# Mange/raingun

Hardware: AMD Instinct MI355X
Metric: Mrays/sec (primary+shadow+secondary) at 3840×2160, depth 5; 1/2/4/8 MI355X (higher is better)
Workload: dtype f64

## Files before the change

include/raingun_debug.h:

```cpp
#ifndef RAINGUN_DEBUG_H
#define RAINGUN_DEBUG_H

#include "raingun.h"

#ifdef __cplusplus
extern "C" {
#endif

rg_status rg_debug_set_path(rg_scene *scene, int32_t path);

typedef struct rg_bvh_info {
    int32_t built;
    int32_t enabled;
    int32_t nodes;
    int32_t leaves;
    int32_t depth;
    float margin;
    float origin_bound;
    int32_t lane_stack;
    int64_t lbuf_bytes;
} rg_bvh_info;
rg_status rg_debug_set_bvh(rg_scene *scene, int32_t enable);
rg_status rg_debug_bvh_info(const rg_scene *scene, rg_bvh_info *info);

// ... 15 lines not shown

rg_status rg_debug_set_host_tile_shape(rg_scene *scene, int32_t tile_wlog);

rg_status rg_debug_set_aa_band_rows(rg_scene *scene, int32_t rows);

rg_status rg_debug_set_aa_adaptive_timing(rg_scene *scene, int32_t enable);
rg_status rg_debug_aa_adaptive_info(const rg_scene *scene, float ms[5], uint32_t *flagged, uint32_t *listed_tiles,
                                    uint32_t *bands_launched);

rg_status rg_debug_set_multi(rg_scene *scene, int32_t mode, int32_t stand_in, int32_t bands, int32_t only_rank);

int rg_debug_gather_noop(const void *send, void *recv, size_t count, int datatype, int root, void *comm,
                         void *stream);

rg_status rg_debug_counters(const rg_scene *scene, uint64_t out[16]);

rg_status rg_debug_counter_words(const rg_scene *scene, int32_t first, int32_t n, uint64_t *out);

rg_status rg_debug_last_plain(const rg_scene *scene, int32_t *plain);

typedef struct rg_shadow_volume_info {
    int32_t built;
    int32_t enabled;
    int32_t g;
    int32_t pad;
    int64_t bytes;
    double build_ms;
    double set_share;
} rg_shadow_volume_info;
rg_status rg_debug_set_shadow_volume(rg_scene *scene, int32_t on);
rg_status rg_debug_shadow_volume_info(const rg_scene *scene, rg_shadow_volume_info *info);
rg_status rg_debug_last_shadow_volume(const rg_scene *scene, int32_t *used);

rg_status rg_debug_set_exact_div(rg_scene *scene, int32_t enable);
rg_status rg_debug_camera_check(const rg_scene *scene, uint32_t width, uint32_t height, double fov,
                                uint64_t *mismatches, int32_t *admitted);

rg_status rg_debug_unscaled_check(const rg_scene *scene, int32_t op, const double *a, const double *b, uint32_t n,
                                  uint64_t *mismatches);

#ifdef __cplusplus
}
#endif

#endif
```

raingun_amd/_abi.py:

```python
from __future__ import annotations

import ctypes as C
import os
from pathlib import Path

PKG_DIR = Path(__file__).resolve().parent
REPO_DIR = PKG_DIR.parent
LIB_PATH = PKG_DIR / "libraingun_hip.so"

RG_OK = 0
RG_ERR_INVALID_ARGUMENT = -1
RG_ERR_PORTRAIT = -2
RG_ERR_AABB_NORMAL = -3
RG_ERR_NAN_DISTANCE = -4
RG_ERR_TRANSMISSION = -5
RG_ERR_TEXTURE = -6
RG_ERR_DEVICE = -10
RG_ERR_OUT_OF_MEMORY = -11
RG_ERR_CANCELLED = -12
RG_ERR_COLLECTIVE = -13
RG_ERR_PENDING = -14

BODY_SPHERE, BODY_PLANE, BODY_DISK, BODY_AABB = 0, 1, 2, 3
COLORATION_COLOR, COLORATION_TEXTURE = 0, 1
# ... 112 lines not shown
    "rg_scene_set_max_depth",
    "rg_render_image",
    "rg_render_tiles_async",
    "rg_render_tiles_pipelined",
    "rg_render_tiles",
    "rg_tiling_rows",
    "rg_render_stream",
    "rg_trace",
    "rg_host_register",
    "rg_host_unregister",
    "rg_scene_release_stream",
    "rg_stream_status",
    "rg_render_multi",
    "rg_render_image_aa",
    "rg_render_aa_async",
    "rg_resolve_box",
    "rg_render_image_aa_adaptive",
    "rg_render_aa_adaptive",
    "rg_edge_mask",
    "rg_camera_look_at",
    "rg_scene_set_camera",
    "rg_render_aov",
    "rg_render_aov_async",
    "rg_scene_set_lens",
    "rg_lens_tables",
)
DEBUG_SYMBOLS = ("rg_debug_set_path", "rg_debug_set_bvh", "rg_debug_bvh_info", "rg_debug_counters",
                 "rg_debug_set_lightbuf", "rg_debug_lightbuf_count",
                 "rg_debug_set_tile_order", "rg_debug_set_lane_depth", "rg_debug_set_image_bands", "rg_debug_set_host_split",
                 "rg_debug_fail_split_a", "rg_debug_set_host_ring", "rg_debug_set_host_tile_shape", "rg_debug_set_multi", "rg_debug_gather_noop",
                 "rg_debug_counter_words", "rg_debug_set_aa_band_rows",
                 "rg_debug_set_aa_adaptive_timing", "rg_debug_aa_adaptive_info", "rg_debug_last_plain",
                 "rg_debug_set_shadow_volume", "rg_debug_shadow_volume_info", "rg_debug_last_shadow_volume",
                 "rg_debug_set_exact_div", "rg_debug_camera_check", "rg_debug_unscaled_check")
FRAMES_SYMBOLS = ("rg_frames_create", "rg_frames_destroy", "rg_frames_step", "rg_frames_flush", "rg_frames_image",
                  "rg_frames_read_image", "rg_frames_status", "rg_frames_set_batch", "rg_frames_set_root_tiles", "rg_comm_id_bytes",
                  "rg_comm_unique_id", "rg_comm_init_rank", "rg_comm_info", "rg_comm_destroy", "rg_comm_gather_fn")
PATH_AUTO, PATH_LIGHT, PATH_HEAVY = -1, 0, 1


class RaingunError(RuntimeError):

    def __init__(self, status: int, what: str = ""):
        self.status = status
        msg = status_string(status) if _LIB is not None else str(status)
        super().__init__(f"{what}: {msg} (status {status})" if what else f"{msg} (status {status})")


_LIB: C.CDLL | None = None


def _declare(lib: C.CDLL) -> None:
    P = C.POINTER
    lib.rg_abi_version.restype = C.c_int32
    lib.rg_status_string.restype = C.c_char_p
    lib.rg_status_string.argtypes = [C.c_int32]
    lib.rg_device_count.restype = C.c_int32
    lib.rg_scene_create.restype = C.c_int32
    lib.rg_scene_create.argtypes = [P(rg_scene_desc), C.c_int32, P(C.c_void_p)]
    lib.rg_scene_destroy.restype = None
    lib.rg_scene_destroy.argtypes = [C.c_void_p]
    lib.rg_scene_set_max_depth.restype = C.c_int32
    lib.rg_scene_set_max_depth.argtypes = [C.c_void_p, C.c_uint32]
    lib.rg_camera_look_at.restype = C.c_int32
    lib.rg_camera_look_at.argtypes = [P(C.c_double), P(C.c_double), P(C.c_double), P(rg_camera)]
    lib.rg_scene_set_camera.restype = C.c_int32
# ... 36 lines not shown
    lib.rg_debug_set_lane_depth.argtypes = [C.c_void_p, C.c_int32]
    lib.rg_debug_set_image_bands.restype = C.c_int32
    lib.rg_debug_set_image_bands.argtypes = [C.c_void_p, C.c_int32]
    if hasattr(lib, "rg_debug_set_host_split"):
        lib.rg_debug_set_host_split.restype = C.c_int32
        lib.rg_debug_set_host_split.argtypes = [C.c_void_p, C.c_int32]
    if hasattr(lib, "rg_debug_set_host_ring"):
        lib.rg_debug_set_host_ring.restype = C.c_int32
        lib.rg_debug_set_host_ring.argtypes = [C.c_void_p] + [C.c_int32] * 5
    if hasattr(lib, "rg_debug_fail_split_a"):
        lib.rg_debug_fail_split_a.restype = C.c_int32
        lib.rg_debug_fail_split_a.argtypes = [C.c_void_p, C.c_int32]
    if hasattr(lib, "rg_debug_set_multi"):
        lib.rg_debug_set_multi.restype = C.c_int32
        lib.rg_debug_set_multi.argtypes = [C.c_void_p, C.c_int32, C.c_int32, C.c_int32, C.c_int32]
    if hasattr(lib, "rg_debug_set_host_tile_shape"):
        lib.rg_debug_set_host_tile_shape.restype = C.c_int32
        lib.rg_debug_set_host_tile_shape.argtypes = [C.c_void_p, C.c_int32]
    lib.rg_debug_counters.restype = C.c_int32
    lib.rg_debug_counters.argtypes = [C.c_void_p, P(C.c_uint64)]
    if hasattr(lib, "rg_debug_counter_words"):
        lib.rg_debug_counter_words.restype = C.c_int32
        lib.rg_debug_counter_words.argtypes = [C.c_void_p, C.c_int32, C.c_int32, P(C.c_uint64)]
    if hasattr(lib, "rg_debug_last_plain"):
        lib.rg_debug_last_plain.restype = C.c_int32
        lib.rg_debug_last_plain.argtypes = [C.c_void_p, P(C.c_int32)]
    if hasattr(lib, "rg_debug_set_shadow_volume"):
        lib.rg_debug_set_shadow_volume.restype = C.c_int32
        lib.rg_debug_set_shadow_volume.argtypes = [C.c_void_p, C.c_int32]
        lib.rg_debug_shadow_volume_info.restype = C.c_int32
        lib.rg_debug_shadow_volume_info.argtypes = [C.c_void_p, P(rg_shadow_volume_info)]
        lib.rg_debug_last_shadow_volume.restype = C.c_int32
        lib.rg_debug_last_shadow_volume.argtypes = [C.c_void_p, P(C.c_int32)]
    if hasattr(lib, "rg_debug_set_exact_div"):
        lib.rg_debug_set_exact_div.restype = C.c_int32
        lib.rg_debug_set_exact_div.argtypes = [C.c_void_p, C.c_int32]
        lib.rg_debug_camera_check.restype = C.c_int32
        lib.rg_debug_camera_check.argtypes = [C.c_void_p, C.c_uint32, C.c_uint32, C.c_double, P(C.c_uint64), P(C.c_int32)]
    if hasattr(lib, "rg_debug_unscaled_check"):
        lib.rg_debug_unscaled_check.restype = C.c_int32
        lib.rg_debug_unscaled_check.argtypes = [C.c_void_p, C.c_int32, C.c_void_p, C.c_void_p, C.c_uint32, P(C.c_uint64)]
    lib.rg_frames_create.restype = C.c_int32
    lib.rg_frames_create.argtypes = [C.c_void_p, C.c_uint32, C.c_uint32, C.c_uint32, C.c_int32, C.c_int32,
                                     C.c_int32, C.c_void_p, C.c_void_p, P(C.c_void_p)]
    lib.rg_frames_destroy.restype = None
    lib.rg_frames_destroy.argtypes = [C.c_void_p]
    lib.rg_frames_step.restype = C.c_int32
    lib.rg_frames_step.argtypes = [C.c_void_p]
    lib.rg_frames_flush.restype = C.c_int32
    lib.rg_frames_flush.argtypes = [C.c_void_p]
    lib.rg_frames_image.restype = C.c_void_p
    lib.rg_frames_image.argtypes = [C.c_void_p]
    lib.rg_frames_read_image.restype = C.c_int32
    lib.rg_frames_read_image.argtypes = [C.c_void_p, C.c_void_p]
    lib.rg_trace.restype = C.c_int32
    lib.rg_trace.argtypes = [C.c_void_p, C.c_void_p, C.c_uint32, C.c_void_p, C.c_void_p]
    lib.rg_host_register.restype = C.c_int32
    lib.rg_host_register.argtypes = [C.c_void_p, C.c_size_t]
    lib.rg_host_unregister.restype = C.c_int32
    lib.rg_host_unregister.argtypes = [C.c_void_p]
    lib.rg_scene_release_stream.restype = C.c_int32
    lib.rg_scene_release_stream.argtypes = [C.c_void_p, C.c_void_p]
    lib.rg_stream_status.restype = C.c_int32
    lib.rg_stream_status.argtypes = [C.c_void_p, C.c_void_p, P(C.c_int32)]
    lib.rg_render_multi.restype = C.c_int32
    lib.rg_render_multi.argtypes = [C.c_void_p, C.c_uint32, C.c_uint32, C.c_int32, C.c_uint32, C.c_void_p,
# ... 100 lines not shown
```

raingun_amd/csrc/rg_capi.hip:

```cpp
#include <hip/hip_runtime.h>

#include <algorithm>
#include <cstring>

#include "../../include/raingun.h"
#include "../../include/raingun_debug.h"
#include "rg_device.h"
#include "rg_exact.h"
#include "rg_internal.h"
#include "rg_launchers.h"

#pragma clang fp contract(off)

#ifndef RG_LANE_MIN_DEPTH
#define RG_LANE_MIN_DEPTH 1
#endif

void rg_image_res_release(rg_image_res &r) {
    rg_bands_release(r);
    if (r.h_frame) (void)hipHostFree(r.h_frame);
    if (r.h_flags) (void)hipHostFree(r.h_flags);
    if (r.h_cancel) (void)hipHostFree(r.h_cancel);
    r = rg_image_res{};
}
// ... 425 lines not shown
    if (!s || !out) return RG_ERR_INVALID_ARGUMENT;
    if (!ok(hipSetDevice(s->device))) return RG_ERR_DEVICE;
    if (!ok(hipStreamSynchronize(s->last->stream)) ||
        !ok(hipMemcpy(out, s->last->last_counters, 16 * sizeof(uint64_t), hipMemcpyDeviceToHost)))
        return RG_ERR_DEVICE;
    return RG_OK;
}

rg_status rg_debug_last_plain(const rg_scene *s, int32_t *plain) {
    if (!s || !plain || !s->last) return RG_ERR_INVALID_ARGUMENT;
    *plain = s->last->last_plain;
    return RG_OK;
}

rg_status rg_debug_set_shadow_volume(rg_scene *s, int32_t on) {
    if (!s || (on != 0 && on != 1)) return RG_ERR_INVALID_ARGUMENT;
    s->shvol_enabled = on != 0;
    return RG_OK;
}

rg_status rg_debug_shadow_volume_info(const rg_scene *s, rg_shadow_volume_info *info) {
    if (!s || !info) return RG_ERR_INVALID_ARGUMENT;
    *info = s->shvol_info;
    info->enabled = s->shvol_info.built && s->shvol_enabled;
    return RG_OK;
}

rg_status rg_debug_last_shadow_volume(const rg_scene *s, int32_t *used) {
    if (!s || !used || !s->last) return RG_ERR_INVALID_ARGUMENT;
    *used = s->last->last_shvol;
    return RG_OK;
}

rg_status rg_debug_set_exact_div(rg_scene *s, int32_t enable) {
    if (!s || (enable != 0 && enable != 1)) return RG_ERR_INVALID_ARGUMENT;
    s->exact_div = enable != 0;
    return RG_OK;
}

rg_status rg_debug_camera_check(const rg_scene *s, uint32_t width, uint32_t height, double fov, uint64_t *mismatches,
                                int32_t *admitted) {
    if (!s || !mismatches || width == 0 || height == 0 || (unsigned long long)width * height >= (1ull << 32))
        return RG_ERR_INVALID_ARGUMENT;
    if (!ok(hipSetDevice(s->device))) return RG_ERR_DEVICE;
    RgKernelArgs a = rg_make_args(s);
    a.width = width;
    a.height = height;
    a.width_d = (double)width;
    a.height_d = (double)height;
    a.aspect = a.width_d / a.height_d;
    a.fov_adjustment = rg_fov_adjustment(fov);
    a.inv_w = 1.0 / a.width_d;
    a.inv_h = 1.0 / a.height_d;
    if (admitted)
        *admitted = rg_recip_div_ok(width) && rg_recip_div_ok(height) && rg_camera_unscaled_ok(a.fov_adjustment, a.aspect);
    unsigned long long *d_bad = nullptr, bad = 0;
    if (!ok(hipMalloc(&d_bad, sizeof bad))) return RG_ERR_OUT_OF_MEMORY;
    rg_status st = RG_OK;
    if (!ok(hipMemset(d_bad, 0, sizeof bad)) || !ok(rg_launch_camera_check(&a, d_bad, nullptr)) ||
        !ok(hipMemcpy(&bad, d_bad, sizeof bad, hipMemcpyDeviceToHost)))
        st = RG_ERR_DEVICE;
    (void)hipFree(d_bad);
    *mismatches = bad;
    return st;
}

// ... 66 lines not shown
```

raingun_amd/csrc/rg_device.h:

```cpp
#pragma once
#include <stdint.h>

#if !defined(__HIP__) && !defined(__HIPCC__)
#define __device__
#define __host__
#define __forceinline__ inline
#endif

#ifdef __HIP_DEVICE_COMPILE__
#define RG_CONST __attribute__((address_space(4)))
#else
#define RG_CONST
#endif
template <class T>
__device__ __forceinline__ const RG_CONST T *rg_cptr(const T *p) { return (const RG_CONST T *)p; }

struct alignas(16) RgSph { double cx, cy, cz, r2; };
struct alignas(16) RgSphF { float cx, cy, cz, r2hi; };
struct alignas(16) RgSphF2 { float cchi, thrp, cc32; int32_t id; };
struct alignas(16) RgPln { double ox, oy, oz, nx, ny, nz, on, pad; };
struct alignas(16) RgDsk { double ox, oy, oz, nx, ny, nz, r, on; };
struct alignas(16) RgBox { double lo[3], hi[3]; };

struct alignas(16) RgBvhNode {
// ... 95 lines not shown
    int32_t nan_scene;
    unsigned long long *err_sticky;
    uint32_t *tile_flags;
    uint32_t frame_seq;
    const uint32_t *cancel;
    uint32_t tile_wlog;
    uint32_t defer_px;
    const double *prim_sx, *prim_sy;
    uint32_t pipelined;
    double width_d, height_d;
    unsigned long long *snap_out;
    uint32_t max_grid_threads;
    uint32_t image_rows;
    uint32_t out_tile_mul, out_tile_add;
    const void *lds_blob;
    const RgLightBufDev *lbuf;
    const uint32_t *lb_start;
    const uint32_t *lb_ent;
    int32_t n_lbuf;
    int32_t lb_cam;
    uint32_t lds_lbuf;
    uint32_t ring_flush, ring_group;
    const uint8_t *px_mask;
    uint32_t tile_limit, px_k, px_w;
    uint32_t plain_veto;
    double inv_w, inv_h;
    uint32_t tiles_x_m, tiles_x_sh, tile_rows_shift, tile_rows_m, tile_rows_sh, rows_identity;
    uint32_t lds_texm, lds_axes, lds_plain_bytes;
    uint32_t camera;
    double cam_eye[3], cam_right[3], cam_up[3], cam_forward[3];
    const uint32_t *shvol;
    uint32_t shvol_g;
    float shvol_inv, shvol_off;
    uint32_t shvol_pad[3];
    uint32_t lens, lens_k;
    double lens_focus, lens_r[3], lens_u[3];
    const double *lens_tab;
    uint32_t lens_pad[2];
};

__host__ __device__ inline uint32_t rg_tile_w(const RgKernelArgs &a) { return 1u << a.tile_wlog; }
__host__ __device__ inline uint32_t rg_tile_h(const RgKernelArgs &a) { return 64u >> a.tile_wlog; }
__host__ __device__ inline uint32_t rg_tiles_x(const RgKernelArgs &a) { return (a.width + rg_tile_w(a) - 1u) >> a.tile_wlog; }
__host__ __device__ inline uint32_t rg_tiles_y(const RgKernelArgs &a) { return (a.out_rows + rg_tile_h(a) - 1u) / rg_tile_h(a); }
__host__ __device__ inline unsigned long long rg_tile_count(const RgKernelArgs &a) {
    return (unsigned long long)rg_tiles_x(a) * rg_tiles_y(a);
}

#define RG_FRAME_BYTES 88

#ifndef RG_RING_FLUSH_SMALL
#define RG_RING_FLUSH_SMALL 4
#endif
#ifndef RG_RING_GROUP_SMALL
#define RG_RING_GROUP_SMALL 1
#endif
#ifndef RG_RING_FLUSH_BIG
#define RG_RING_FLUSH_BIG 8
#endif
#ifndef RG_RING_GROUP_BIG
#define RG_RING_GROUP_BIG 8
#endif
#ifndef RG_RING_BIG_TILES
#define RG_RING_BIG_TILES 50000u
#endif
#ifndef RG_MULTI_LIGHT_ONE
#define RG_MULTI_LIGHT_ONE 1
#endif
#ifndef RG_LB
#define RG_LB 3
#endif
#ifndef RG_LB_SMALL
#define RG_LB_SMALL 2
#endif
#ifndef RG_LB_ONE
#define RG_LB_ONE 1
#endif
#ifndef RG_PLAIN_SHVOL
#define RG_PLAIN_SHVOL 1
#endif
#ifndef RG_PLAIN_SHVOL_SPHERES
#define RG_PLAIN_SHVOL_SPHERES 1
#endif
#ifndef RG_PLAIN_SHVOL_PLANES
#define RG_PLAIN_SHVOL_PLANES 1
#endif
#ifndef RG_HEAVY_WPS
#define RG_HEAVY_WPS 3
#endif
#define RG_BVH_MAX_WAVES 16
#ifndef RG_HEAVY_SCENE_BODIES
#define RG_HEAVY_SCENE_BODIES 32
#endif

#define RG_PATH_AUTO -1
#define RG_PATH_LIGHT 0
#define RG_PATH_HEAVY 1

__host__ __device__ __forceinline__ bool rg_heavy_path(const RgKernelArgs &a) {
    bool heavy = a.n_sph + a.n_pln + a.n_dsk + a.n_box >= RG_HEAVY_SCENE_BODIES;
    if (a.path != RG_PATH_AUTO) heavy = a.path == RG_PATH_HEAVY;
    if (a.n_lights > RG_LB) heavy = true;
    return heavy;
}

#define RG_COUNTER_WORDS (16 + 16 * 16 + 16)
#define RG_DONE_WORD (16 + 16 * 16)
```

raingun_amd/csrc/rg_internal.h:

```cpp
#pragma once
#include <hip/hip_runtime.h>

#include <cstddef>
#include <cstring>
#include <initializer_list>
#include <memory>
#include <vector>

#include "../../include/raingun.h"
#include "../../include/raingun_debug.h"
#include "rg_bands.h"
#include "rg_copy_pool.h"
#include "rg_device.h"
#include "rg_lightbuf_ray.h"
#include "rg_tile_deal.h"

inline bool ok(hipError_t e) { return e == hipSuccess; }

struct rg_launch_ctx {
    hipStream_t stream = nullptr;
    unsigned long long *counters = nullptr;
    int cur = 0;
    unsigned long long *last_counters = nullptr;
    int last_plain = 0;
// ... 99 lines not shown
    int device = 0;
    double fov = 90.0;
    float def[3] = {0, 0, 0};
    uint32_t max_depth = 10;
    int32_t n_sph = 0, n_pln = 0, n_dsk = 0, n_box = 0, n_bodies = 0, n_lights = 0, n_textures = 0;
    bool nan_scene = false;
    std::vector<void *> allocations;
    RgSph *sph = nullptr;
    double *sph_cc = nullptr;
    RgSphF *sphf = nullptr;
    RgSphF2 *sphf2 = nullptr;
    int32_t path = RG_PATH_AUTO;
    int32_t *sph_id = nullptr, *pln_id = nullptr, *dsk_id = nullptr, *box_id = nullptr;
    RgPln *pln = nullptr;
    RgDsk *dsk = nullptr;
    RgBox *box = nullptr;
    RgBodyDev *bodies = nullptr;
    RgMatDev *mats = nullptr;
    RgLightDev *lights = nullptr;
    RgTexDev *texs = nullptr;
    RgBvhNode *nodes = nullptr;
    int32_t n_nodes = 0;
    int32_t lane_stack = 0;
    int32_t lane_min_depth = 1;
    bool bvh_enabled = true;
    RgLightBufDev *lbuf = nullptr;
    uint32_t *lb_start = nullptr, *lb_ent = nullptr;
    int32_t n_lbuf = 0;
    int32_t lb_cam = -1;
    int32_t n_lbdesc = 0;
    bool lbuf_enabled = true;
    uint32_t *shvol = nullptr;
    bool shvol_enabled = true;
    rg_shadow_volume_info shvol_info{};
    float shvol_inv = 0.0f, shvol_off = 0.0f;
    bool exact_div = true;
    bool has_camera = false;
    rg_camera camera{};
    rg_lens lens{0.0, 1.0};
    float bvh_obound = 0.0f;
    double bvh_rbound = 0.0, bvh_margin = 0.0, bvh_extent = 0.0;
    rg_bvh_info bvh_info{};
    int tile_order = -1;
    int image_bands = 0;
    int host_split_pct = 0;
    mutable int split_fail_a = 0;
    int ring_flush_small = RG_RING_FLUSH_SMALL, ring_group_small = RG_RING_GROUP_SMALL;
    int ring_flush_big = RG_RING_FLUSH_BIG, ring_group_big = RG_RING_GROUP_BIG;
    bool multi_light_one = RG_MULTI_LIGHT_ONE != 0;
    int host_tile_wlog = RG_HOST_TILE_WLOG;
    bool host_tile_forced = false;
    int multi_mode = 0;
    bool multi_stand_in = false;
    int multi_bands = 0;
    int multi_only_rank = -1;
    std::shared_ptr<const rg_host_tables> host;
    std::vector<RgTexDev> tex_desc;
    void *lds_blob = nullptr;
    uint32_t lds_blob_layout[14] = {};
    mutable std::vector<rg_launch_ctx *> ctxs;
    mutable rg_launch_ctx *last = nullptr;
    mutable rg_image_res img;
    int aa_band_rows = 0;
    mutable rg_aa_res aa;
    mutable rg_multi_res *multi = nullptr;
    mutable std::vector<rg_frames *> frames;
// ... 81 lines not shown
```

raingun_amd/csrc/rg_k_math.h:

```cpp
#pragma once
#include <hip/hip_runtime.h>
#include <cstdint>

#include "rg_device.h"
#include "rg_exact.h"

#pragma clang fp contract(off)

namespace rgk {

constexpr double SHADOW_BIAS = 1e-13;
constexpr float PI_F = 3.14159265358979323846f;

enum : int { MODE_CLOSEST = 0, MODE_SHADOW = 1, MODE_DONE = 2, MODE_WAIT = 3, MODE_SHADOW_H = 4 };
enum : int { FR_REFL = 0, FR_REFR_T = 1, FR_REFR_R = 2, FR_REFR_TASK = 4, FR_REFR_WAIT = 5 };

struct V3 { double x, y, z; };
struct C3 { float r, g, b; };

__device__ __forceinline__ V3 v3(double x, double y, double z) { return V3{x, y, z}; }
__device__ __forceinline__ V3 add(V3 a, V3 b) { return v3(a.x + b.x, a.y + b.y, a.z + b.z); }
__device__ __forceinline__ V3 sub(V3 a, V3 b) { return v3(a.x - b.x, a.y - b.y, a.z - b.z); }
__device__ __forceinline__ V3 scl(V3 a, double s) { return v3(a.x * s, a.y * s, a.z * s); }
__device__ __forceinline__ V3 neg(V3 a) { return v3(-a.x, -a.y, -a.z); }
// ... 76 lines not shown
__device__ __forceinline__ C3 cadd(C3 a, C3 b) { return c3(a.r + b.r, a.g + b.g, a.b + b.b); }
__device__ __forceinline__ C3 cmul(C3 a, C3 b) { return c3(a.r * b.r, a.g * b.g, a.b * b.b); }
__device__ __forceinline__ C3 cscl(C3 a, float s) { return c3(a.r * s, a.g * s, a.b * s); }
__device__ __forceinline__ C3 cclamp(C3 a) {
    return c3(fmaxf(fminf(a.r, 1.0f), 0.0f), fmaxf(fminf(a.g, 1.0f), 0.0f), fmaxf(fminf(a.b, 1.0f), 0.0f));
}

__device__ __forceinline__ uint32_t f32_to_u8(float v) {
    if (!(v > 0.0f)) return 0u;
    if (v >= 255.0f) return 255u;
    return (uint32_t)v;
}
__device__ __forceinline__ int32_t f32_to_i32(float v) {
    if (v != v) return 0;
    if (v >= 2147483648.0f) return 2147483647;
    if (v < -2147483648.0f) return (-2147483647 - 1);
    return (int32_t)v;
}

__device__ __forceinline__ double readlane_d(double v, int l) {
    const unsigned long long b = (unsigned long long)__double_as_longlong(v);
    const uint32_t lo = (uint32_t)__builtin_amdgcn_readlane((int)(uint32_t)b, l);
    const uint32_t hi = (uint32_t)__builtin_amdgcn_readlane((int)(uint32_t)(b >> 32), l);
    return __longlong_as_double((long long)(((unsigned long long)hi << 32) | lo));
}

#define RG_REGION_BASE 144
enum : int {
    RGR_LOOP = 0, RGR_PRIM, RGR_PRIM_SPH_TAIL, RGR_PRIM_PLANE_DIV, RGR_GETCOLOR, RGR_NORMAL_SPHERE,
    RGR_BATCH, RGR_TEXEL, RGR_UV_SPHERE, RGR_UV_PLANE, RGR_LIGHT_SPH, RGR_REFRACT, RGR_SHADE, RGR_UNWIND,
    RGR_UNWIND_STEP, RGR_TILE_FETCH, RGR_Q_CLOSEST, RGR_Q_SHADOW, RGR_SH_GROUP, RGR_SH_TAIL, RGR_SH_PLANE,
    RGR_SH_PLANE_DIV, RGR_QC_GROUP, RGR_QC_TAIL, RGR_QC_PLANE, RGR_PRIM_GROUP, RGR_PRIM_PLANE, RGR_DISK, RGR_BOX,
    RGR_PUSH_REFL, RGR_PUSH_REFR, RGR_UNWIND_REFRT, RGR_ERROR, RGR_SH_PAIR, RGR_PRIM_PAIR, RGR_QC_PAIR,
    RGR_WALK, RGR_WALK_LEAF, RGR_LB_SHADOW, RGR_COUNT
};
static_assert(RG_REGION_BASE + 2 * RGR_COUNT <= 16 + 16 * 15, "region counters stay below tile-queue head 15");
#ifdef RG_REGION_STATS
#define RG_REGION(k)                                                                                  \
    do {                                                                                              \
        const unsigned long long m_ = __ballot(1);                                                    \
        if ((int)(threadIdx.x & 63u) == __builtin_ffsll((long long)m_) - 1) {                         \
            atomicAdd(&a.counters[RG_REGION_BASE + 2 * (k)], 1ull);                                   \
            atomicAdd(&a.counters[RG_REGION_BASE + 2 * (k) + 1], (unsigned long long)__builtin_popcountll(m_)); \
        }                                                                                             \
    } while (0)
#else
#define RG_REGION(k) do { } while (0)
#endif

__device__ __forceinline__ void raise_error(const RgKernelArgs &a, uint32_t pixel, int status) {
    RG_REGION(RGR_ERROR);
    unsigned long long key = ((unsigned long long)pixel << 8) | (unsigned long long)(-status);
    atomicMax(&a.counters[3], ~key);
    if (a.err_sticky) atomicMax(a.err_sticky, ~key);
}

}
```

raingun_amd/csrc/rg_render_kernel.h:

```cpp
#pragma once
#include <hip/hip_runtime.h>

#include "../../include/raingun.h"
#include "rg_camera.h"
#include "rg_device.h"
#include "rg_k_bvh.h"
#include "rg_k_diag.h"
#include "rg_k_frames.h"
#include "rg_k_intersect.h"
#include "rg_k_math.h"
#include "rg_k_pool.h"
#include "rg_k_shade.h"
#include "rg_k_trace.h"
#include "rg_lens.h"
#include "rg_render_cfg.h"
#include "rg_shadow_vol_cell.h"

#pragma clang fp contract(off)

using namespace rgk;

#ifndef RG_NQ
#define RG_NQ 8
#endif
// ... 142 lines not shown
#endif
    [[maybe_unused]] const unsigned long long t_kernel = RG_CLOCK();
#ifdef RG_WAVE_TIMES
    const unsigned long long t_staged = wall_clock64();
#endif
    const uint32_t twlog = K::host_frames ? a.tile_wlog : 3u, twmask = (1u << twlog) - 1u, th = 64u >> twlog;
    const uint32_t tiles_x = (a.width + twmask) >> twlog;
    const uint32_t ntiles = tiles_x * ((a.out_rows + th - 1u) / th);
    const C3 def = c3(a.def[0], a.def[1], a.def[2]);
    const int max_depth = (int)a.max_depth;
    [[maybe_unused]] const bool use_ring = RING > 0 && a.defer_px;
    [[maybe_unused]] const uint32_t ring_n = RING > 0 ? (a.ring_flush ? min(a.ring_flush, (uint32_t)(RING > 0 ? RING : 1)) : (uint32_t)RING) : 1u;
    [[maybe_unused]] const uint32_t ring_g = RING > 0 ? (a.ring_group ? min(a.ring_group, ring_n) : ring_n) : 1u;
    [[maybe_unused]] auto flush_ring = [&]() {
        for (uint32_t k = 0; k < nring; ++k) {
            const uint32_t tile = ring_tile[rw][k];
            const uint32_t ty = tile / tiles_x, tx = tile - ty * tiles_x;
            const uint32_t x = (tx << twlog) + ((uint32_t)lane & twmask);
            const uint32_t orow = ty * th + ((uint32_t)lane >> twlog);
            if (x < a.width && orow < a.out_rows) {
                const uint32_t row = a.image_rows ? out_row_to_y(a, orow) : out_row_of(a, orow);
                if (row != 0xFFFFFFFFu) a.rgba[(size_t)row * a.width + x] = ring_px[rw][k][lane];
            }
        }
        if (a.tile_flags) {
            __builtin_amdgcn_fence(__ATOMIC_RELEASE, "");
            if ((uint32_t)lane < nring)
                __hip_atomic_store(&a.tile_flags[ring_tile[rw][lane]], a.frame_seq, __ATOMIC_RELAXED,
                                   __HIP_MEMORY_SCOPE_SYSTEM);
        }
        nring = 0;
    };
    uint32_t n_prim = 0, n_shadow = 0, n_sec = 0;
    FrameStack<K::array_frames> stk;
    stk.init(a);

    uint32_t qi = blockIdx.x % RG_NQ, qtried = 0;
    int mode = MODE_DONE;
    Ray q;
    ShadowBatch<LB> sb;
    uint32_t occl_full = 0u;
    [[maybe_unused]] uint32_t shw = 0u;
    int qdepth = 0;
    V3 hp = v3(0, 0, 0), hn = v3(0, 0, 0);
    int hb = 0, hdepth = 0, li = 0;
    int nfan = 0;
    uint32_t fan_lanes = 0u;
    uint32_t fan_bits = 0u;
    C3 fin = c3(0, 0, 0), bcol = c3(0, 0, 0), ret = def;
    int sp = 0;
    Closest c;
    closest_init(c);
    bool have_result = false;
    uint32_t occl = 0u;
    size_t oidx = 0;
    uint32_t pixel = 0;
    int task = -1;
    bool tiles_left = true;
    [[maybe_unused]] uint32_t pf_k = 0u;
    [[maybe_unused]] bool pf_valid = false;
    uint32_t my_tile = 0xFFFFFFFFu;
    [[maybe_unused]] uint32_t tiles_taken = 0;
    [[maybe_unused]] bool counted = false;
#ifdef RG_TILE_TIMES
    uint32_t cur_tile = 0xFFFFFFFFu;
    unsigned long long t_tile = 0, t_query = 0;
// ... 466 lines not shown
                        sy = a.prim_sy[y];
                    } else {
                        sensor_div(a, x, y, sx, sy);
                    }
                    if constexpr (K::camera) {
                        double dir[3];
                        if constexpr (K::lens) {
                            double org[3];
                            rg_lens_ray(a.cam_eye, a.cam_right, a.cam_up, a.cam_forward, sx, sy, x, y, a.lens_k,
                                        a.width / a.lens_k, a.lens_focus, a.lens_r, a.lens_u,
                                        a.lens_tab + 2u * rg_lens_points_offset(a.lens_k), a.lens_tab + 2u * RG_LENS_POINTS,
                                        org, dir);
                            q.o = v3(org[0], org[1], org[2]);
                        } else {
                        rg_camera_direction(a.cam_right, a.cam_up, a.cam_forward, sx, sy, dir);
                        q.o = v3(a.cam_eye[0], a.cam_eye[1], a.cam_eye[2]);
                        }
                        q.d = v3(dir[0], dir[1], dir[2]);
                        n_prim++;
                        have_result = false;
                    } else {
                    q.o = v3(0.0, 0.0, 0.0);
                    if constexpr (fast_camera) q.d = normalize_camera(sx, sy);
                    else q.d = normalize(v3(sx, sy, -1.0));
                    n_prim++;
                    closest_init(c);
                    trace_primary<F32F, BVH, PLAIN>(a, src, q.d, c);
                    have_result = true;
                    }
                    mode = MODE_CLOSEST;
                    qdepth = 0;
                    task = -1;
                }
                continue;
            }
        }
        if constexpr (K::shadow_fan) {
            const int want = mode == MODE_SHADOW ? min(a.n_lights - li - 1, RG_SHADOW_FAN) : 0;
            unsigned long long owners = __ballot(want > 0);
            if (owners != 0ull) {
                unsigned long long idle = __ballot(mode == MODE_DONE);
                while (owners != 0ull && idle != 0ull) {
                    const int o = __builtin_ctzll(owners);
                    owners &= owners - 1ull;
                    const int w = __builtin_amdgcn_readlane(want, o);
                    const int oli = __builtin_amdgcn_readlane(li, o);
                    const int ohd = __builtin_amdgcn_readlane(hdepth, o);
                    const uint32_t opix = (uint32_t)__builtin_amdgcn_readlane((int)pixel, o);
                    const V3 ohp = v3(readlane_d(hp.x, o), readlane_d(hp.y, o), readlane_d(hp.z, o));
                    const V3 oso = v3(readlane_d(q.o.x, o), readlane_d(q.o.y, o), readlane_d(q.o.z, o));
                    uint32_t packed = 0u;
                    int k = 0;
                    for (; k < w && idle != 0ull; ++k) {
                        const int hl = __builtin_ctzll(idle);
                        idle &= idle - 1ull;
                        packed |= (uint32_t)hl << (6 * k);
                        if (lane == hl) {
                            hp = ohp;
                            q.o = oso;
                            hdepth = ohd;
                            pixel = opix;
                            light_dir_dist<UL>(T.lights[oli + 1 + k], hp, sb.d[0], sb.ld[0]);
                            li = oli + 1 + k;
                            mode = MODE_SHADOW_H;
                        }
                    }
// ... 136 lines not shown
    }
    if constexpr (RING > 0) {
        if (use_ring) flush_ring();
    }
#ifdef RG_TILE_TIMES
    if (cur_tile != 0xFFFFFFFFu && lane == 0 && a.rgb) {
        a.rgb[cur_tile] = (float)(wall_clock64() - t_tile) * 0.01f;
        a.rgb[ntiles + cur_tile] = (float)tile_iters;
        a.rgb[2 * ntiles + cur_tile] = (float)(t_tile & 0xFFFFFFull);
        a.rgb[3 * ntiles + cur_tile] = (float)t_query * 0.01f;
    }
#endif

    RG_STAT(14, RG_CLOCK() - t_kernel);
    RG_STAT(15, 1);
#ifdef RG_WAVE_TIMES
    if (lane == 0 && a.rgb) {
        const unsigned long long t_end = wall_clock64();
        uint32_t *wt = reinterpret_cast<uint32_t *>(a.rgb) + 4u * (blockIdx.x * (blockDim.x / 64u) + (threadIdx.x >> 6));
        wt[0] = (uint32_t)t_wave0;
        wt[1] = (uint32_t)(t_staged - t_wave0);
        wt[2] = (uint32_t)(t_end - t_wave0);
        wt[3] = wt_tiles;
    }
#endif
#ifdef RG_BVH_STATS
    if (lane >= 4 && lane < 16) atomicAdd(&a.counters[lane], rg_stat_lds[(threadIdx.x >> 6) % RG_BVH_MAX_WAVES][lane]);
#endif
    unsigned long long p64 = wave_sum(n_prim), s64 = wave_sum(n_shadow), q64 = wave_sum(n_sec);
    if (lane == 0) {
        if (p64) atomicAdd(&a.counters[0], p64);
        if (s64) atomicAdd(&a.counters[1], s64);
        if (q64) atomicAdd(&a.counters[2], q64);
        if (a.snap_out) {
            __builtin_amdgcn_s_waitcnt(0);
            const unsigned long long waves = (unsigned long long)gridDim.x * (blockDim.x >> 6);
            if (atomicAdd(&a.counters[RG_DONE_WORD], 1ull) == waves - 1ull) {
#pragma unroll
                for (int k = 0; k < 4; ++k)
                    a.snap_out[k] = __hip_atomic_load(&a.counters[k], __ATOMIC_RELAXED, __HIP_MEMORY_SCOPE_AGENT);
            }
        }
    }
}
```

raingun_amd/csrc/rg_scene.hip:

```cpp
#include <hip/hip_runtime.h>

#include <algorithm>
#include <cmath>
#include <cstring>
#include <memory>
#include <new>
#include <vector>

#include "../../include/raingun.h"
#include "../../include/raingun_debug.h"
#include "rg_bvh.h"
#include "rg_camera.h"
#include "rg_device.h"
#include "rg_exact.h"
#include "rg_lens.h"
#include "rg_lightbuf.h"
#include "rg_shadow_vol.h"
#include "rg_internal.h"

#pragma clang fp contract(off)

#ifndef RG_BVH_MIN_SPHERES
#define RG_BVH_MIN_SPHERES 16
#endif
// ... 170 lines not shown
    const bool lane = bvh && rg_heavy_path(a) && s->lane_stack > 0 && s->lane_min_depth < 1 << 20;
    a.lane_stack = lane ? s->lane_stack : 0;
    a.lane_min_depth = lane ? s->lane_min_depth : 1 << 30;
    a.lds_lstack_bytes = lane ? ((uint32_t)(a.lane_stack + 1) * 4u) * 256u * RG_HEAVY_WPS : 0u;
    auto al16 = [](uint32_t v) { return (v + 15u) & ~15u; };
    a.lds_sphf = a.lds_lstack_bytes;
    a.lds_sph = a.lds_sphf + (uint32_t)s->n_sph * (uint32_t)(sizeof(RgSphF) + sizeof(RgSphF2));
    a.lds_cc = a.lds_sph + (uint32_t)s->n_sph * (uint32_t)sizeof(RgSph);
    a.lds_nodes = al16(a.lds_cc + (uint32_t)s->n_sph * 8u);
    a.lds_pln = a.lds_nodes + (uint32_t)a.n_nodes * (uint32_t)sizeof(RgBvhNode);
    a.lds_dsk = a.lds_pln + (uint32_t)s->n_pln * (uint32_t)sizeof(RgPln);
    a.lds_box = a.lds_dsk + (uint32_t)s->n_dsk * (uint32_t)sizeof(RgDsk);
    a.lds_lights = al16(a.lds_box + (uint32_t)s->n_box * (uint32_t)sizeof(RgBox));
    a.lds_texs = a.lds_lights + (uint32_t)s->n_lights * (uint32_t)sizeof(RgLightDev);
    a.lds_lbuf = al16(a.lds_texs + (uint32_t)s->n_textures * (uint32_t)sizeof(RgTexDev));
    a.lds_bodies = a.lds_lbuf + (a.lbuf ? (uint32_t)s->n_lbdesc * (uint32_t)sizeof(RgLightBufDev) : 0u);
    a.lds_hot_bytes = a.lds_bodies;
    a.lds_mats = a.lds_bodies + (uint32_t)s->n_bodies * (uint32_t)sizeof(RgBodyDev);
    a.lds_total_bytes = a.lds_mats + (uint32_t)s->n_bodies * (uint32_t)sizeof(RgMatDev);
    a.lds_texm = a.lds_total_bytes;
    a.lds_axes = a.lds_texm + (uint32_t)s->n_textures * (uint32_t)sizeof(RgTexMagic);
    a.lds_plain_bytes = a.lds_axes + (uint32_t)s->n_bodies * (uint32_t)sizeof(RgPlnAxes);
    a.def[0] = s->def[0];
    a.def[1] = s->def[1];
    a.def[2] = s->def[2];
    a.max_depth = s->max_depth;
    a.fov_adjustment = fov_adjustment(s->fov);
    a.tile_wlog = 3;
    const bool shvol = RG_PLAIN_SHVOL != 0 && s->shvol_enabled && s->shvol != nullptr;
    a.shvol = shvol ? s->shvol : nullptr;
    a.shvol_g = shvol ? (uint32_t)s->shvol_info.g : 0u;
    a.shvol_inv = s->shvol_inv;
    a.shvol_off = s->shvol_off;
    return a;
}

double rg_fov_adjustment(double fov) { return fov_adjustment(fov); }

bool rg_scene_heavy(const rg_scene *s) {
    RgKernelArgs a;
    std::memset(&a, 0, sizeof a);
    a.n_sph = s->n_sph;
    a.n_pln = s->n_pln;
    a.n_dsk = s->n_dsk;
    a.n_box = s->n_box;
    a.path = s->path;
    a.n_lights = s->n_lights;
    return rg_heavy_path(a);
}

const void *rg_lds_blob_for(const rg_scene *s, const RgKernelArgs &a) {
    const uint32_t layout[14] = {a.lds_sphf, a.lds_sph, a.lds_cc, a.lds_nodes, a.lds_pln, a.lds_dsk, a.lds_box,
                                 a.lds_bodies, a.lds_mats, a.lds_lights, a.lds_texs, a.lds_total_bytes,
                                 (uint32_t)a.n_nodes, (uint32_t)a.n_sph};
    rg_scene *m = const_cast<rg_scene *>(s);
    if (m->lds_blob && std::memcmp(layout, m->lds_blob_layout, sizeof layout) == 0) return m->lds_blob;
    if (!s->host || a.lds_total_bytes == 0 || a.lds_total_bytes % 16u != 0u || a.lds_plain_bytes % 16u != 0u)
        return nullptr;
    const rg_host_tables &h = *s->host;
    std::vector<unsigned char> img(a.lds_plain_bytes, 0);
    auto put = [&](uint32_t off, const void *src, size_t bytes) {
        if (bytes && off + bytes <= img.size()) std::memcpy(img.data() + off, src, bytes);
    };
    put(a.lds_sphf, h.sphf.data(), h.sphf.size() * sizeof(RgSphF));
    put(a.lds_sphf + (uint32_t)(h.sphf.size() * sizeof(RgSphF)), h.sphf2.data(), h.sphf2.size() * sizeof(RgSphF2));
    put(a.lds_sph, h.sph.data(), h.sph.size() * sizeof(RgSph));
// ... 25 lines not shown
    if (m->lds_blob) {
        m->allocations.push_back(m->lds_blob);
    }
    m->lds_blob = p;
    std::memcpy(m->lds_blob_layout, layout, sizeof layout);
    return p;
}

rg_status rg_scene_replica(const rg_scene *src, int32_t device, rg_scene **out) {
    *out = nullptr;
    if (!src->host) return RG_ERR_INVALID_ARGUMENT;
    rg_scene *s = new (std::nothrow) rg_scene();
    if (!s) return RG_ERR_OUT_OF_MEMORY;
    s->device = device;
    copy_scalars(s, src);
    rg_sync_settings(s, src);
    s->host = src->host;
    if (!ok(hipSetDevice(device))) { release(s); return RG_ERR_DEVICE; }
    rg_status st = upload_tables(s, *src->host);
    if (st == RG_OK && !(s->last = rg_ctx_for(s, nullptr))) st = RG_ERR_OUT_OF_MEMORY;
    if (st != RG_OK) { release(s); return st; }
    *out = s;
    return RG_OK;
}

void rg_scene_free(rg_scene *s) { release(s); }

void rg_sync_settings(rg_scene *dst, const rg_scene *src) {
    dst->max_depth = src->max_depth;
    dst->path = src->path;
    dst->bvh_enabled = src->bvh_enabled;
    dst->lbuf_enabled = src->lbuf_enabled;
    dst->shvol_enabled = src->shvol_enabled;
    dst->exact_div = src->exact_div;
    dst->has_camera = src->has_camera;
    dst->camera = src->camera;
    dst->lens = src->lens;
    dst->lane_min_depth = src->lane_min_depth;
    dst->tile_order = src->tile_order;
    dst->ring_flush_small = src->ring_flush_small;
    dst->ring_group_small = src->ring_group_small;
    dst->ring_flush_big = src->ring_flush_big;
    dst->ring_group_big = src->ring_group_big;
}

extern "C" {

rg_status rg_scene_create(const rg_scene_desc *d, int32_t device, rg_scene **out) {
    if (!d || !out) return RG_ERR_INVALID_ARGUMENT;
    *out = nullptr;
    if ((d->n_bodies && !d->bodies) || (d->n_lights && !d->lights) || (d->n_textures && !d->textures))
        return RG_ERR_INVALID_ARGUMENT;
    int ndev = 0;
    if (hipGetDeviceCount(&ndev) != hipSuccess || device < 0 || device >= ndev) return RG_ERR_DEVICE;
    bool nan_scene = false;
    for (uint32_t i = 0; i < d->n_bodies; ++i) {
        const rg_body &b = d->bodies[i];
        if (b.kind > RG_BODY_AABB || b.material.coloration > RG_COLORATION_TEXTURE ||
            b.material.surface > RG_SURFACE_REFRACTIVE)
            return RG_ERR_INVALID_ARGUMENT;
        if (b.material.coloration == RG_COLORATION_TEXTURE) {
            int32_t t = b.material.texture;
            if (t < 0 || (uint32_t)t >= d->n_textures || !d->textures[t].rgba || d->textures[t].width == 0 ||
                d->textures[t].height == 0 || d->textures[t].width > 0x7fffffffu || d->textures[t].height > 0x7fffffffu)
                return RG_ERR_TEXTURE;
        }
// ... 261 lines not shown
```

raingun_amd/scene.py:

```python
from __future__ import annotations

import ctypes as C
import os
from dataclasses import dataclass, field
from pathlib import Path
from typing import Callable, List, Optional, Sequence, Union

import numpy as np

from . import _abi, aov
from .camera import Camera, Lens
from .color import Color



class SceneError(ValueError):
    """The YAML does not deserialise into a Scene (serde_yaml's Err)."""


@dataclass
class Texture:
    path: str
    image: np.ndarray
    x_offset: float
# ... 235 lines not shown
        _abi.check(_abi.lib().rg_debug_set_multi(self.handle, int(mode), 1 if stand_in else 0, int(bands),
                                                 int(only_rank)))

    def set_host_ring(self, flush_small: int = -1, group_small: int = -1, flush_big: int = -1, group_big: int = -1,
                      multi_light_one: int = -1) -> None:
        _abi.check(_abi.lib().rg_debug_set_host_ring(self.handle, int(flush_small), int(group_small), int(flush_big),
                                                     int(group_big), int(multi_light_one)))

    def set_host_split(self, pct: int) -> None:
        _abi.check(_abi.lib().rg_debug_set_host_split(self.handle, int(pct)))

    def set_host_tile_shape(self, tile_wlog: int) -> None:
        _abi.check(_abi.lib().rg_debug_set_host_tile_shape(self.handle, int(tile_wlog)))

    def last_plain(self) -> bool:
        plain = C.c_int32(-1)
        _abi.check(_abi.lib().rg_debug_last_plain(self.handle, C.byref(plain)))
        return plain.value == 1

    def set_shadow_volume(self, on: bool) -> None:
        _abi.check(_abi.lib().rg_debug_set_shadow_volume(self.handle, 1 if on else 0))

    def shadow_volume_info(self) -> dict:
        info = _abi.rg_shadow_volume_info()
        _abi.check(_abi.lib().rg_debug_shadow_volume_info(self.handle, C.byref(info)))
        return {"built": bool(info.built), "enabled": bool(info.enabled), "g": info.g, "bytes": info.bytes,
                "build_ms": info.build_ms, "set_share": info.set_share}

    def last_shadow_volume(self) -> bool:
        used = C.c_int32(-1)
        _abi.check(_abi.lib().rg_debug_last_shadow_volume(self.handle, C.byref(used)))
        return used.value == 1

    def set_exact_div(self, enable: bool) -> None:
        _abi.check(_abi.lib().rg_debug_set_exact_div(self.handle, 1 if enable else 0))

    def camera_check(self, width: int, height: int, fov: float):
        bad, admitted = C.c_uint64(0), C.c_int32(-1)
        _abi.check(_abi.lib().rg_debug_camera_check(self.handle, int(width), int(height), float(fov), C.byref(bad),
                                                    C.byref(admitted)))
        return int(bad.value), admitted.value == 1

    def unscaled_check(self, op: int, a, b=None) -> int:
        import numpy as np

        a = np.ascontiguousarray(a, dtype=np.float64)
        bp = None
        if b is not None:
            b = np.ascontiguousarray(b, dtype=np.float64)
            assert b.shape == a.shape
            bp = b.ctypes.data_as(C.c_void_p)
        bad = C.c_uint64(0)
        _abi.check(_abi.lib().rg_debug_unscaled_check(self.handle, int(op), a.ctypes.data_as(C.c_void_p), bp, a.size,
                                                      C.byref(bad)))
        return int(bad.value)

    def bvh_info(self) -> _abi.rg_bvh_info:
        info = _abi.rg_bvh_info()
        _abi.check(_abi.lib().rg_debug_bvh_info(self.handle, C.byref(info)))
        return info

    def set_max_depth(self, depth: int) -> None:
        _abi.check(_abi.lib().rg_scene_set_max_depth(self.handle, int(depth)))

    def set_camera(self, camera: Optional[Camera]) -> None:
        if camera is None:
# ... 216 lines not shown
```

Before: 159,800.

## Shade whole waves at first hit when every lane hits a diffuse surface

Adds a fast path in the PLAIN render kernel. When every lane in a wave hits a diffuse surface (or a reflector at depth 1), the wave computes normals, texture, light terms and one batched shadow trace inline, writes the pixel and finishes. This skips the general frame-stack and secondary-ray machinery for simple waves. It costs extra code size and register pressure in the kernel, plus a wave-wide check on every primary hit. A debug toggle and a counter are added so the path can be switched off and its use counted.

```diff
diff --git a/include/raingun_debug.h b/include/raingun_debug.h
--- a/include/raingun_debug.h
+++ b/include/raingun_debug.h
@@ -71,6 +71,9 @@
 rg_status rg_debug_shadow_volume_info(const rg_scene *scene, rg_shadow_volume_info *info);
 rg_status rg_debug_last_shadow_volume(const rg_scene *scene, int32_t *used);
 
+rg_status rg_debug_set_first_hit_tiles(rg_scene *scene, int32_t on);
+rg_status rg_debug_last_first_hit_tiles(const rg_scene *scene, uint64_t *tiles);
+
 rg_status rg_debug_set_exact_div(rg_scene *scene, int32_t enable);
 rg_status rg_debug_camera_check(const rg_scene *scene, uint32_t width, uint32_t height, double fov,
                                 uint64_t *mismatches, int32_t *admitted);
diff --git a/raingun_amd/_abi.py b/raingun_amd/_abi.py
--- a/raingun_amd/_abi.py
+++ b/raingun_amd/_abi.py
@@ -168,6 +168,7 @@
                  "rg_debug_counter_words", "rg_debug_set_aa_band_rows",
                  "rg_debug_set_aa_adaptive_timing", "rg_debug_aa_adaptive_info", "rg_debug_last_plain",
                  "rg_debug_set_shadow_volume", "rg_debug_shadow_volume_info", "rg_debug_last_shadow_volume",
+                 "rg_debug_set_first_hit_tiles", "rg_debug_last_first_hit_tiles",
                  "rg_debug_set_exact_div", "rg_debug_camera_check", "rg_debug_unscaled_check")
 FRAMES_SYMBOLS = ("rg_frames_create", "rg_frames_destroy", "rg_frames_step", "rg_frames_flush", "rg_frames_image",
                   "rg_frames_read_image", "rg_frames_status", "rg_frames_set_batch", "rg_frames_set_root_tiles", "rg_comm_id_bytes",
@@ -270,6 +271,11 @@
         lib.rg_debug_shadow_volume_info.argtypes = [C.c_void_p, P(rg_shadow_volume_info)]
         lib.rg_debug_last_shadow_volume.restype = C.c_int32
         lib.rg_debug_last_shadow_volume.argtypes = [C.c_void_p, P(C.c_int32)]
+    if hasattr(lib, "rg_debug_set_first_hit_tiles"):
+        lib.rg_debug_set_first_hit_tiles.restype = C.c_int32
+        lib.rg_debug_set_first_hit_tiles.argtypes = [C.c_void_p, C.c_int32]
+        lib.rg_debug_last_first_hit_tiles.restype = C.c_int32
+        lib.rg_debug_last_first_hit_tiles.argtypes = [C.c_void_p, P(C.c_uint64)]
     if hasattr(lib, "rg_debug_set_exact_div"):
         lib.rg_debug_set_exact_div.restype = C.c_int32
         lib.rg_debug_set_exact_div.argtypes = [C.c_void_p, C.c_int32]
diff --git a/raingun_amd/csrc/rg_capi.hip b/raingun_amd/csrc/rg_capi.hip
--- a/raingun_amd/csrc/rg_capi.hip
+++ b/raingun_amd/csrc/rg_capi.hip
@@ -481,6 +481,17 @@
     return RG_OK;
 }
 
+rg_status rg_debug_set_first_hit_tiles(rg_scene *s, int32_t on) {
+    if (!s || (on != 0 && on != 1)) return RG_ERR_INVALID_ARGUMENT;
+    s->first_hit_enabled = on != 0;
+    return RG_OK;
+}
+
+rg_status rg_debug_last_first_hit_tiles(const rg_scene *s, uint64_t *tiles) {
+    if (!s || !tiles || !s->last) return RG_ERR_INVALID_ARGUMENT;
+    return rg_debug_counter_words(s, RG_FIRST_HIT_WORD, 1, tiles);
+}
+
 rg_status rg_debug_set_exact_div(rg_scene *s, int32_t enable) {
     if (!s || (enable != 0 && enable != 1)) return RG_ERR_INVALID_ARGUMENT;
     s->exact_div = enable != 0;
diff --git a/raingun_amd/csrc/rg_device.h b/raingun_amd/csrc/rg_device.h
--- a/raingun_amd/csrc/rg_device.h
+++ b/raingun_amd/csrc/rg_device.h
@@ -151,7 +151,10 @@
     const uint32_t *shvol;
     uint32_t shvol_g;
     float shvol_inv, shvol_off;
-    uint32_t shvol_pad[3];
+    union {
+        uint32_t shvol_pad[3];
+        uint32_t first_hit_off;
+    };
     uint32_t lens, lens_k;
     double lens_focus, lens_r[3], lens_u[3];
     const double *lens_tab;
@@ -204,6 +207,9 @@
 #ifndef RG_PLAIN_SHVOL_PLANES
 #define RG_PLAIN_SHVOL_PLANES 1
 #endif
+#ifndef RG_PLAIN_FIRST_HIT
+#define RG_PLAIN_FIRST_HIT 1
+#endif
 #ifndef RG_HEAVY_WPS
 #define RG_HEAVY_WPS 3
 #endif
@@ -225,3 +231,4 @@
 
 #define RG_COUNTER_WORDS (16 + 16 * 16 + 16)
 #define RG_DONE_WORD (16 + 16 * 16)
+#define RG_FIRST_HIT_WORD (RG_DONE_WORD + 1)
diff --git a/raingun_amd/csrc/rg_internal.h b/raingun_amd/csrc/rg_internal.h
--- a/raingun_amd/csrc/rg_internal.h
+++ b/raingun_amd/csrc/rg_internal.h
@@ -155,6 +155,7 @@
     bool lbuf_enabled = true;
     uint32_t *shvol = nullptr;
     bool shvol_enabled = true;
+    bool first_hit_enabled = true;
     rg_shadow_volume_info shvol_info{};
     float shvol_inv = 0.0f, shvol_off = 0.0f;
     bool exact_div = true;
diff --git a/raingun_amd/csrc/rg_k_math.h b/raingun_amd/csrc/rg_k_math.h
--- a/raingun_amd/csrc/rg_k_math.h
+++ b/raingun_amd/csrc/rg_k_math.h
@@ -132,7 +132,7 @@
     RGR_UNWIND_STEP, RGR_TILE_FETCH, RGR_Q_CLOSEST, RGR_Q_SHADOW, RGR_SH_GROUP, RGR_SH_TAIL, RGR_SH_PLANE,
     RGR_SH_PLANE_DIV, RGR_QC_GROUP, RGR_QC_TAIL, RGR_QC_PLANE, RGR_PRIM_GROUP, RGR_PRIM_PLANE, RGR_DISK, RGR_BOX,
     RGR_PUSH_REFL, RGR_PUSH_REFR, RGR_UNWIND_REFRT, RGR_ERROR, RGR_SH_PAIR, RGR_PRIM_PAIR, RGR_QC_PAIR,
-    RGR_WALK, RGR_WALK_LEAF, RGR_LB_SHADOW, RGR_COUNT
+    RGR_WALK, RGR_WALK_LEAF, RGR_LB_SHADOW, RGR_FIRST_HIT, RGR_COUNT
 };
 static_assert(RG_REGION_BASE + 2 * RGR_COUNT <= 16 + 16 * 15, "region counters stay below tile-queue head 15");
 #ifdef RG_REGION_STATS
diff --git a/raingun_amd/csrc/rg_render_kernel.h b/raingun_amd/csrc/rg_render_kernel.h
--- a/raingun_amd/csrc/rg_render_kernel.h
+++ b/raingun_amd/csrc/rg_render_kernel.h
@@ -198,6 +198,7 @@
         nring = 0;
     };
     uint32_t n_prim = 0, n_shadow = 0, n_sec = 0;
+    [[maybe_unused]] uint32_t n_first_hit = 0;
     FrameStack<K::array_frames> stk;
     stk.init(a);
 
@@ -730,6 +731,95 @@
                     qdepth = 0;
                     task = -1;
                 }
+                if constexpr (PLAIN && RG_PLAIN_FIRST_HIT != 0) {
+                    const bool hit = alive && c.id >= 0;
+                    const int surf = hit ? T.mats[c.id].surface : RG_SURFACE_DIFFUSE;
+                    const bool simple = !alive || (!c.nan && (surf == RG_SURFACE_DIFFUSE ||
+                                                              (surf == RG_SURFACE_REFLECTING && 1 >= max_depth)));
+                    if (!a.first_hit_off && !__any(!simple)) {
+                        RG_REGION(RGR_FIRST_HIT);
+                        static_assert(!K::camera, "the primary rays of a PLAIN kernel leave the origin");
+                        float pp[LB], lin[LB];
+                        C3 bc = c3(0.0f, 0.0f, 0.0f);
+                        float refl = 0.0f, rr = 0.0f;
+                        [[maybe_unused]] uint32_t fw = 0u;
+                        bool bail = false;
+#pragma unroll
+                        for (int l = 0; l < LB; ++l) pp[l] = lin[l] = 0.0f;
+                        if (hit) {
+                            const RgBodyDev b = T.bodies[c.id];
+                            const RgMatDev m = T.mats[c.id];
+                            const V3 h = add(q.o, scl(q.d, c.t));
+                            V3 n;
+                            if (!surface_normal(b, h, n)) bail = true;
+                            const bool textured = m.coloration != RG_COLORATION_COLOR;
+                            uint32_t texel = 0u;
+                            if (textured) texel = texel_fetch_plain(T.texs, PT, m, b, c.id, h);
+                            else bc = c3(m.color[0], m.color[1], m.color[2]);
+                            refl = m.albedo_pi;
+                            rr = m.reflectivity;
+                            q.o = add(h, scl(n, SHADOW_BIAS));
+                            if constexpr (SHV) {
+                                fw = RG_SHVOL_ALL;
+                                if (a.shvol) {
+                                    const int cell = rg_shvol_cell((float)q.o.x, (float)q.o.y, (float)q.o.z, a.shvol_inv,
+                                                                   a.shvol_off, (int)a.shvol_g);
+                                    const uint32_t w = a.shvol[cell >= 0 ? cell : 0];
+                                    if (cell >= 0) fw = w;
+                                }
+                            }
+#pragma unroll
+                            for (int l = 0; l < LB; ++l) {
+                                const RgLightDev L = T.lights[l];
+                                light_dir_dist<UL>(L, h, sb.d[l], sb.ld[l]);
+                                pp[l] = fmaxf((float)dot(n, sb.d[l]), 0.0f);
+                                lin[l] = light_intensity(L, h);
+                                bail |= ray_exotic(q.o, sb.d[l]);
+                            }
+                            if (textured) bc = texel_color(texel);
+                        }
+                        if (__any(bail)) {
+                            q.o = v3(0.0, 0.0, 0.0);
+                        } else {
+                            q.d = v3(0.0, 0.0, 0.0);
+                            closest_init(c);
+                            uint32_t focc = 0u;
+                            [[maybe_unused]] uint32_t smask = ~0u, pmask = ~0u;
+                            bool walk = true;
+                            if constexpr (SHV) {
+                                if (a.shvol) {
+                                    const uint32_t wm = wave_or(hit ? fw : 0u);
+                                    smask = wm & 0xFFFFu;
+                                    pmask = wm >> 16;
+                                    walk = wm != 0u;
+                                }
+                            }
+                            C3 fret = def;
+                            if (hit) {
+                                if (walk) trace_shadow<LB, PLAIN, SHV>(a, src, q.o, sb, (1u << LB) - 1u, focc, smask, pmask);
+                                n_shadow += (uint32_t)LB;
+                                C3 acc = c3(0.0f, 0.0f, 0.0f);
+#pragma unroll
+                                for (int l = 0; l < LB; ++l) {
+                                    const RgLightDev L = T.lights[l];
+                                    const float inten = !((focc >> l) & 1u) ? lin[l] : 0.0f;
+                                    const float power = pp[l] * inten;
+                                    const C3 lc = cscl(cscl(c3(L.color[0], L.color[1], L.color[2]), power), refl);
+                                    acc = cadd(acc, cmul(bc, lc));
+                                }
+                                const C3 dcol = cclamp(acc);
+                                fret = surf == RG_SURFACE_DIFFUSE ? dcol : cadd(cscl(dcol, 1.0f - rr), cscl(def, rr));
+                            }
+                            if (alive) {
+                                a.rgba[oidx] = f32_to_u8(fret.r * 255.0f) | (f32_to_u8(fret.g * 255.0f) << 8) |
+                                               (f32_to_u8(fret.b * 255.0f) << 16) | 0xFF000000u;
+                            }
+                            mode = MODE_DONE;
+                            have_result = false;
+                            ++n_first_hit;
+                        }
+                    }
+                }
                 continue;
             }
         }
@@ -932,6 +1022,9 @@
         if (p64) atomicAdd(&a.counters[0], p64);
         if (s64) atomicAdd(&a.counters[1], s64);
         if (q64) atomicAdd(&a.counters[2], q64);
+        if constexpr (PLAIN && RG_PLAIN_FIRST_HIT != 0) {
+            if (n_first_hit) atomicAdd(&a.counters[RG_FIRST_HIT_WORD], (unsigned long long)n_first_hit);
+        }
         if (a.snap_out) {
             __builtin_amdgcn_s_waitcnt(0);
             const unsigned long long waves = (unsigned long long)gridDim.x * (blockDim.x >> 6);
diff --git a/raingun_amd/csrc/rg_scene.hip b/raingun_amd/csrc/rg_scene.hip
--- a/raingun_amd/csrc/rg_scene.hip
+++ b/raingun_amd/csrc/rg_scene.hip
@@ -226,6 +226,7 @@
     a.shvol_g = shvol ? (uint32_t)s->shvol_info.g : 0u;
     a.shvol_inv = s->shvol_inv;
     a.shvol_off = s->shvol_off;
+    a.first_hit_off = s->first_hit_enabled ? 0u : 1u;
     return a;
 }
 
@@ -317,6 +318,7 @@
     dst->bvh_enabled = src->bvh_enabled;
     dst->lbuf_enabled = src->lbuf_enabled;
     dst->shvol_enabled = src->shvol_enabled;
+    dst->first_hit_enabled = src->first_hit_enabled;
     dst->exact_div = src->exact_div;
     dst->has_camera = src->has_camera;
     dst->camera = src->camera;
diff --git a/raingun_amd/scene.py b/raingun_amd/scene.py
--- a/raingun_amd/scene.py
+++ b/raingun_amd/scene.py
@@ -291,6 +291,14 @@
         _abi.check(_abi.lib().rg_debug_last_shadow_volume(self.handle, C.byref(used)))
         return used.value == 1
 
+    def set_first_hit_tiles(self, on: bool) -> None:
+        _abi.check(_abi.lib().rg_debug_set_first_hit_tiles(self.handle, 1 if on else 0))
+
+    def last_first_hit_tiles(self) -> int:
+        tiles = C.c_uint64(0)
+        _abi.check(_abi.lib().rg_debug_last_first_hit_tiles(self.handle, C.byref(tiles)))
+        return int(tiles.value)
+
     def set_exact_div(self, enable: bool) -> None:
         _abi.check(_abi.lib().rg_debug_set_exact_div(self.handle, 1 if enable else 0))
 
```

Result: faster. 172,100, median of 6 (+7.7%).
